# urbste/OpenImuCameraCalibrator

Measured on AMD Instinct MI355X. Metric: residual+Jacobian blocks/sec; wall-clock per LM iter, GoPro9 full calib, higher is better.
Workload: dtype f64

## Files before the change

openimucameracalibrator_amd/csrc/kernels_bcr.hip:

```cpp
#include <hip/hip_runtime.h>
#include <mutex>
#include <unordered_map>
#include "oicc_device.h"
#include "lm_decide.h"
#include "lm_launch.h"
#include "lm_retract.h"
#include "bcr_chain_body.h"
#include "../../include/oicc_hip.h"

namespace oicc {


struct BcrArgs {
  double* D;
  double* F;
  double* S;
  double* Lf;
  double* Mc;
  double* x;
  int32_t* fail;
  long long* prof;
  int n, a, Pb, rtf, LD;
  int delay;
  int o, s, p, m, pn;
// ... 8 lines not shown
#define BCR_RETURN_IF_DONE(A) do { if ((A).ctl != nullptr && (A).ctl->done != 0) return; } while (0)

__device__ __forceinline__ void bcr_lds_barrier() { asm volatile("s_waitcnt lgkmcnt(0)\n\ts_barrier" ::: "memory"); }
typedef double bcr_v4d __attribute__((ext_vector_type(4)));
typedef double bcr_v2d __attribute__((ext_vector_type(2)));

__device__ __forceinline__ void tri10(int t, int& xt, int& yt) {
  xt = t < 1 ? 0 : (t < 3 ? 1 : (t < 6 ? 2 : 3));
  yt = t - (xt * (xt + 1)) / 2;
}

struct BcrNoIdle { __device__ __forceinline__ void operator()() const {} };
template <int LD, class Idle = BcrNoIdle>
__device__ __forceinline__ void bcr_corner_solve(double* C, double* da, int* failp, int a, int tid, int wave, int lane, Idle idle = Idle()) {
  const int a1 = a + 1;
  if (a1 <= 16) {
    if (wave == 0) {
      double av[16], dinv = 0.0;
#pragma unroll
      for (int c = 0; c < 16; ++c) av[c] = (c < a && lane < a1 && lane >= c) ? C[c * LD + lane] : 0.0;
      bool bad = false;
#pragma unroll
      for (int c = 0; c < 16; ++c) {
        if (c < a) {
          const double piv = bcr_readlane(av[c], c);
          bad |= !(piv > 0.0);
          const double y0 = __builtin_amdgcn_rsq(piv);
          const double g0 = piv * y0, h0 = 0.5 * y0;
          const double r0 = fma(-g0, h0, 0.5);
          const double g1 = fma(g0, r0, g0), h1 = fma(h0, r0, h0);
          const double r1 = fma(-g1, h1, 0.5);
          const double u = (av[c] + av[c]) * h1;
          const double l = fma(u, r1, u);
          av[c] = l;
          if (lane == c) { const double y1 = h1 + h1; dinv = fma(y1, r1, y1); }
#pragma unroll
          for (int c2 = c + 1; c2 < 16; ++c2) {
            const double lc2 = bcr_readlane(l, c2);
            av[c2] = fma(-l, lc2, av[c2]);
          }
        }
      }
#pragma unroll
      for (int c = 0; c < 16; ++c) if (c < a && lane < a1 && lane >= c) C[c * LD + lane] = av[c];
      double lt[16];
#pragma unroll
      for (int q = 0; q < 16; ++q) lt[q] = (q < a && lane < q) ? C[lane * LD + q] : 0.0;
      double z = lane < a ? C[lane * LD + a] : 0.0, xq_mine = 0.0;
#pragma unroll
      for (int q = 15; q >= 0; --q) {
        if (q < a) {
          const double xq = bcr_readlane(z * dinv, q);
          if (lane == q) xq_mine = xq;
          z = fma(-lt[q], xq, z);
        }
      }
      if (lane < a) da[lane] = xq_mine;
      if (bad && lane == 0) *failp = 1;
    } else idle();
    __syncthreads();
    return;
  }
  if (wave == 0) {
    bool bad = false;
    for (int c = 0; c < a; ++c) {
      double* col = C + c * LD;
      const double mine = lane < a1 ? col[lane] : 0.0;
      double piv = bcr_readlane(mine, c);
      if (!(piv > 0.0)) { bad = true; piv = 1.0; }
      const double d = sqrt(piv);
      const double l = lane == c ? d : (lane > c ? mine / d : 0.0);
      if (lane >= c && lane < a1) col[lane] = l;
      for (int c2 = c + 1; c2 < a; ++c2) {
        const double l2 = bcr_readlane(l, c2);
        if (lane >= c2 && lane < a1) C[c2 * LD + lane] -= l * l2;
      }
    }
    if (bad && lane == 0) *failp = 1;
    double z = lane < a ? C[lane * LD + a] : 0.0;
    const double dc = lane < a ? 1.0 / C[lane * LD + lane] : 0.0;
    double xq_mine = 0.0;
    for (int q = a - 1; q >= 0; --q) {
      const double xq = bcr_readlane(z * dc, q);
      if (lane == q) xq_mine = xq;
      const double l = lane < q ? C[lane * LD + q] : 0.0;
      z = fma(-l, xq, z);
    }
    if (lane < a) da[lane] = xq_mine;
  } else idle();
  __syncthreads();
}

constexpr int kBackWaves = 8;
constexpr int kInvWaves = 16;
constexpr int kInvLD = 145;
constexpr int kInvMsDoubles = 3 * kChainStripDoubles;
constexpr int kInvDgRow = 128;

template <int XT>
__device__ __forceinline__ bcr_v4d bcri_z_tile(const double* W, int yt, int li, int lq) {
  constexpr int LD = kInvLD, K0 = 4 * XT, NK = 16 - K0;
  const double* py = W + lq * LD + 64 + 16 * yt + li;
  const double* px = W + lq * LD + 64 + 16 * XT + li;
  double vy[NK], vx[NK];
#pragma unroll
  for (int kk = 0; kk < NK; ++kk) { vy[kk] = py[4 * (K0 + kk) * LD]; vx[kk] = px[4 * (K0 + kk) * LD]; }
  asm volatile("" ::: "memory");
  bcr_v4d g = {0.0, 0.0, 0.0, 0.0}, g2 = {0.0, 0.0, 0.0, 0.0};
#pragma unroll
  for (int kk = 0; kk < NK; kk += 2) {
    g = __builtin_amdgcn_mfma_f64_16x16x4f64(vy[kk], vx[kk], g, 0, 0, 0);
    g2 = __builtin_amdgcn_mfma_f64_16x16x4f64(vy[kk + 1], vx[kk + 1], g2, 0, 0, 0);
  }
  g += g2;
  return g;
}

constexpr int kBackRows = 192 / kBackWaves;
struct BcrBackX {
  const double* xl; const double* xr; const double* xa;
  bool hasL, hasR;
  __device__ __forceinline__ double at(int r, int a) const {
    return r < 64 ? (hasL ? xl[r] : 0.0) : (r < 128 ? (hasR ? xr[r - 64] : 0.0) : (r < 128 + a ? xa[r - 128] : 0.0));
  }
};
__device__ __forceinline__ void bcri_back_rows(const double* Tg, int a, bool hasL, bool hasR, int w, int lane, double (&lv)[kBackRows], double& yv) {
#pragma unroll
  for (int k = 0; k < kBackRows; ++k) {
    const int r = w + kBackWaves * k;
    const bool ok = r < 128 + a && (hasL || r >= 64) && (hasR || r < 64 || r >= 128);
    lv[k] = ok ? Tg[r * 64 + lane] : 0.0;
  }
  yv = w == 0 ? Tg[(128 + a) * 64 + lane] : 0.0;
}
__device__ __forceinline__ double bcri_back_body(const double (&lv)[kBackRows], double yv, const BcrBackX& X, int a, double* part, bool active, int w, int lane) {
  if (active) {
    double sum = 0.0;
#pragma unroll
    for (int k = 0; k < kBackRows; ++k) { const int r = w + kBackWaves * k; sum = fma(lv[k], X.at(r, a), sum); }
    part[w * 64 + lane] = sum;
  }
  __syncthreads();
  double acc = 0.0;
  if (active && w == 0) {
#pragma unroll
    for (int ww = 0; ww < kBackWaves; ++ww) acc += part[ww * 64 + lane];
  }
  return yv - acc;
}

template <bool LAST, bool ZLDS, bool FOLD>
__device__ __forceinline__ void bcri_tail(const BcrArgs& A, double* W, double* da, int* failp, const double* Fs, const double* Cs, double* Zg, int tid, int wave, int lane, bool report, double* x0s) {
  static_assert(!FOLD || LAST, "the folded level follows the last block");
  constexpr int LD = kInvLD, NW = kInvWaves, NT = 64 * NW, FLD = 65;
  const int li = lane & 15, lq = lane >> 4;
  const int a = A.a, a1 = a + 1;
  const bool shared_writer = !FOLD || blockIdx.x == 0;
  double ttop[16], ytop = 0.0;
#pragma unroll
  for (int k = 0; k < 16; ++k) ttop[k] = 0.0;
  if (LAST && (A.top_l >= 0 || A.top_r >= 0)) {
    const int64_t ru64 = (int64_t)(192 + a1) * 64;
    const double* Tr = A.Lf + (A.top_r >= 0 ? A.top_r : 0) * ru64 + 4096;
    const double* Tl = A.Lf + (A.top_l >= 0 ? A.top_l : 0) * ru64 + 4096;
#pragma unroll
    for (int k = 0; k < 4; ++k) {
      const int r = wave + NW * k;
      if (A.top_r >= 0) { ttop[k] = Tr[r * 64 + lane]; if (r < A.a) ttop[4 + k] = Tr[(128 + r) * 64 + lane]; }
      if (A.top_l >= 0) { ttop[8 + k] = Tl[(64 + r) * 64 + lane]; if (r < A.a) ttop[12 + k] = Tl[(128 + r) * 64 + lane]; }
    }
    if (wave == 0 && A.top_r >= 0) ytop = Tr[(128 + A.a) * 64 + lane];
    if (wave == 1 && A.top_l >= 0) ytop = Tl[(128 + A.a) * 64 + lane];
    asm volatile("" ::: "memory");
  }
  for (int t = wave; t < 10; t += NW) {
    int xt, yt; tri10(t, xt, yt);
    const bcr_v4d g = xt == 0 ? bcri_z_tile<0>(W, yt, li, lq) : (xt == 1 ? bcri_z_tile<1>(W, yt, li, lq) : (xt == 2 ? bcri_z_tile<2>(W, yt, li, lq) : bcri_z_tile<3>(W, yt, li, lq)));
#pragma unroll
    for (int r = 0; r < 4; ++r) {
      const int x = 16 * xt + li, y = 16 * yt + lq + 4 * r;
      if (LAST || ZLDS) { W[y * LD + x] = g[r]; if (xt != yt) W[x * LD + y] = g[r]; }
      else { Zg[y * 64 + x] = g[r]; if (xt != yt) Zg[x * 64 + y] = g[r]; }
    }
  }
  __syncthreads();
  if (!LAST) {
    if (report && tid == 0 && *failp) atomicOr(A.fail, 1);
    return;
  }
  const int rtf = A.rtf;
  if (wave < 4 * rtf) {
    const int t = wave >> 2, w = wave & 3;
    const double* pf = Fs + lq * FLD + 16 * t + li;
    const double* pz = W + lq * LD + 16 * w + li;
    double vf[16], vz[16];
#pragma unroll
    for (int kk = 0; kk < 16; ++kk) { vf[kk] = pf[4 * kk * FLD]; vz[kk] = pz[4 * kk * LD]; }
    asm volatile("" ::: "memory");
    bcr_v4d tq = {0.0, 0.0, 0.0, 0.0};
#pragma unroll
    for (int kk = 0; kk < 16; ++kk) tq = __builtin_amdgcn_mfma_f64_16x16x4f64(vf[kk], vz[kk], tq, 0, 0, 0);
#pragma unroll
    for (int r = 0; r < 4; ++r) W[(16 * w + li) * LD + 64 + 16 * t + lq + 4 * r] = tq[r];
  }
  __syncthreads();
  if (wave < (rtf * (rtf + 1)) / 2) {
    int t1 = 0, u = wave; while (u >= t1 + 1) { u -= t1 + 1; ++t1; }
    const int t2 = u;
    const double* pt = W + lq * LD + 64 + 16 * t1 + li;
    const double* pf = Fs + lq * FLD + 16 * t2 + li;
    double vt[16], vf[16];
#pragma unroll
    for (int kk = 0; kk < 16; ++kk) { vt[kk] = pt[4 * kk * LD]; vf[kk] = pf[4 * kk * FLD]; }
    asm volatile("" ::: "memory");
    bcr_v4d g = {0.0, 0.0, 0.0, 0.0};
#pragma unroll
    for (int kk = 0; kk < 16; ++kk) g = __builtin_amdgcn_mfma_f64_16x16x4f64(vf[kk], vt[kk], g, 0, 0, 0);
#pragma unroll
    for (int r = 0; r < 4; ++r) { const int q1 = 16 * t1 + li, q2 = 16 * t2 + lq + 4 * r; if (q1 < a1 && q2 < a1) W[q2 * LD + q1] = Cs[q1 * a1 + q2] - g[r]; }
  }
  double lv[kBackRows], yv = 0.0;
#pragma unroll
  for (int k = 0; k < kBackRows; ++k) lv[k] = 0.0;
  constexpr int BW0 = NW - kBackWaves;
  int fi = 0; bool f_hasL = false, f_hasR = false;
  if (FOLD) {
    const int kp = 2 * (int)blockIdx.x + A.p;
    fi = A.o + kp * A.s; f_hasL = kp > 0; f_hasR = kp < A.m - 1;
  }
  __syncthreads();
  bcr_corner_solve<LD>(W, da, failp, a, tid, wave, lane, [&]() {
    if (FOLD && wave >= BW0) {
      bcri_back_rows(A.Lf + (int64_t)fi * (192 + a1) * 64 + 4096, a, f_hasL, f_hasR, wave - BW0, lane, lv, yv);
      asm volatile("" ::: "memory");
    }
  });
  if (shared_writer) for (int q = tid; q < a; q += NT) A.x[A.Pb + q] = da[q];
  if (wave == 0) {
    const double* tc = W + lane * LD + 64;
    double v = tc[a];
    for (int q = 0; q < a; q += 8) {
      double t8[8], d8[8];
#pragma unroll
      for (int k = 0; k < 8; ++k) { const bool ok = q + k < a; t8[k] = ok ? tc[q + k] : 0.0; d8[k] = ok ? da[q + k] : 0.0; }
#pragma unroll
      for (int k = 0; k < 8; ++k) v = fma(-t8[k], d8[k], v);
    }
    const int gi = A.last * 64 + lane;
    if (shared_writer && gi < A.Pb) A.x[gi] = v;
    x0s[lane] = gi < A.Pb ? v : 0.0;
  }
  __syncthreads();
  if (shared_writer && tid == 0 && *failp) atomicOr(A.fail, 1);
  if (A.top_l >= 0 || A.top_r >= 0) {
    double sum_r = 0.0, sum_l = 0.0;
#pragma unroll
    for (int k = 0; k < 4; ++k) {
      const int r = wave + NW * k;
      const double xn = x0s[r], xa = r < a ? da[r] : 0.0;
      sum_r = fma(ttop[k], xn, sum_r);     sum_r = fma(ttop[4 + k], xa, sum_r);
      sum_l = fma(ttop[8 + k], xn, sum_l); sum_l = fma(ttop[12 + k], xa, sum_l);
    }
    W[wave * 64 + lane] = sum_r;
    W[(NW + wave) * 64 + lane] = sum_l;
    __syncthreads();
    if (wave < 2) {
      const int blk = wave == 0 ? A.top_r : A.top_l;
      double acc = 0.0;
#pragma unroll
      for (int w = 0; w < NW; ++w) acc += W[(wave * NW + w) * 64 + lane];
      const int gi = blk * 64 + lane;
      const bool ok = blk >= 0 && gi < A.Pb;
      if (shared_writer && ok) A.x[gi] = ytop - acc;
      if (FOLD) x0s[64 * (1 + wave) + lane] = ok ? ytop - acc : 0.0;
    }
    if (FOLD) {
      __syncthreads();
      auto x_of = [&](int blk) -> const double* { return blk == A.last ? x0s : (blk == A.top_r ? x0s + 64 : x0s + 128); };
      BcrBackX X;
      X.hasL = f_hasL; X.hasR = f_hasR; X.xl = x_of(fi - A.s); X.xr = x_of(fi + A.s); X.xa = da;
      const double xv = bcri_back_body(lv, yv, X, a, W + 2 * NW * 64, wave >= BW0, wave - BW0, lane);
      const int gi = fi * 64 + lane;
      if (wave == BW0 && gi < A.Pb) A.x[gi] = xv;
    }
  }
}


struct BcrNoPark { __device__ __forceinline__ void operator()(double*) const {} };
template <bool LAST, bool PROF, bool ZLDS = false, bool FOLD = false, class LoadD, class Park = BcrNoPark>
__device__ __forceinline__ void bcri_invert_body(const BcrArgs& A, const int i, LoadD load_d, const bool report = true, Park park = Park()) {
  constexpr int LD = kInvLD, NW = kInvWaves, NT = 64 * NW, NTILE = 20, SLOTS = (NTILE + NW - 1) / NW, RU = 128, NAW = 3, FLD = 65;
  static_assert(NW == 16, "the corner phases of block 0 take one tile per wave");
  extern __shared__ __attribute__((aligned(16))) double lds[];
  const int tid = threadIdx.x, lane = tid & 63;
  const int wave = __builtin_amdgcn_readfirstlane(tid >> 6);
  const int li = lane & 15, lq = lane >> 4;
  double* const W = lds;
  double* const da = W + 64 * LD;
  int* const failp = reinterpret_cast<int*>(da + 64);
  double* const ms = da + 64 + 8;
  static_assert(kInvMsDoubles >= NAW * kChainStripDoubles && (kChainStripDoubles * 8) % 16 == 0 && kInvMsDoubles >= 256 && ((64 * LD + 64 + 8) * 8) % 16 == 0, "ms");
  double* const Fs = ms + kInvMsDoubles;
  double* const Cs = Fs + 64 * FLD;
  const int a1 = A.a + 1;
  double* Zg = A.Lf + (int64_t)i * (192 + a1) * 64;
  const double* Fg = A.F + (int64_t)i * 64 * a1;
  const double* Sf = (LAST && A.side != 0) ? Zg + 4096 : nullptr;
  const double* Sm = (LAST && A.side != 0) ? Zg + 4096 + 64 * a1 : nullptr;
  const bool prof = PROF && A.prof != nullptr && blockIdx.x == 0 && wave == 0;
  long long pc[8] = {0, 0, 0, 0, 0, 0, 0, 0};
  long long tprev = prof ? clock64() : 0;
#define BCR_MARK(k) do { if (PROF && prof) { const long long tn_ = clock64(); pc[k] += tn_ - tprev; tprev = tn_; } } while (0)
  if (tid == 0) *failp = 0;
  {
    constexpr int PER = 4096 / NT;
    double gd[PER], gf[PER], gc[PER];
#pragma unroll
    for (int k = 0; k < PER; ++k) {
      const int e = tid + k * NT;
      gd[k] = load_d(e);
      if (LAST) { const int c = e >> 6, q = e & 63; gf[k] = q < a1 ? Fg[c * a1 + q] + (Sf != nullptr ? Sf[c * a1 + q] : 0.0) : 0.0; }
      if (LAST) gc[k] = e < a1 * a1 ? A.Mc[e] + (Sm != nullptr ? Sm[e] : 0.0) : 0.0;
    }
#pragma unroll
    for (int k = 0; k < PER; ++k) {
      const int e = tid + k * NT;
      const int c = e >> 6, r = e & 63;
      W[c * LD + r] = r >= c ? gd[k] : 0.0;
      if (c < 16 && r < 16) W[c * LD + kInvDgRow + r] = r >= c ? gd[k] : 0.0;
      W[c * LD + 64 + r] = r == c ? 1.0 : 0.0;
      if (LAST) Fs[c * FLD + r] = gf[k];
      if (LAST && e < a1 * a1) Cs[e] = gc[k];
    }
    park(Fs);
  }
  __syncthreads();
  int t_rt[SLOTS], t_ct[SLOTS]; bool t_ok[SLOTS];
  bcr_v4d acc[SLOTS];
#pragma unroll
  for (int k = 0; k < SLOTS; ++k) {
    const int t = wave + NW * k;
    t_ok[k] = t < NTILE;
    int xt, yt; tri10(t < 10 ? t : (t < NTILE ? t - 10 : 0), xt, yt);
    if (t < 10) { t_rt[k] = xt; t_ct[k] = yt; } else { t_rt[k] = 4 + yt; t_ct[k] = xt; }
    const double* src = W + (16 * t_ct[k] + lq) * LD + 16 * t_rt[k] + li;
    acc[k][0] = src[0]; acc[k][1] = src[4 * LD]; acc[k][2] = src[8 * LD]; acc[k][3] = src[12 * LD];
  }
  BCR_MARK(0);
  const int prow = 16 + wave * 48 + (lane - 16);
  for (int p = 0; p < 4; ++p) {
    const int j0 = 16 * p;
    if (wave < NAW) {
      const int rho = lane < 16 ? j0 + lane : prow;
      const bool act = lane < 16 || (rho >= j0 + 16 && rho < RU && !(rho >= 64 && rho - 64 > j0 + 15));
      if (A.delay > 0 && wave > 0) for (int k = 0; k < A.delay; ++k) __builtin_amdgcn_s_sleep(16);
      const double* colp = W + j0 * LD + (lane < 16 ? kInvDgRow + lane : (act ? rho : 0));
      double av[16];
#pragma unroll
      for (int c = 0; c < 16; ++c) av[c] = colp[c * LD];
      if (PROF && prof) { asm volatile("s_waitcnt lgkmcnt(0)" ::: "memory"); }
      BCR_MARK(6);
      const bool bad = bcr_chain_panel<kChainSchedule>(av, ms + wave * kChainStripDoubles + lane, ms + wave * kChainStripDoubles);
      if (PROF && prof) { asm volatile("s_nop 0" :: "v"(av[15])); }
      BCR_MARK(7);
      if (act && (lane >= 16 || wave == 0)) {
        double* cp = W + j0 * LD + rho;
#pragma unroll
        for (int c = 0; c < 16; ++c) cp[c * LD] = av[c];
      }
      if (bad && lane == 0) *failp = 1;
    }
    BCR_MARK(1);
    bcr_lds_barrier();
    BCR_MARK(2);
    if (p < 3) {
#pragma unroll
      for (int k = 0; k < SLOTS; ++k) {
        if (t_ok[k] && t_ct[k] > p && (t_rt[k] < 4 || t_rt[k] - 4 <= p)) {
          const double* pa = W + (j0 + lq) * LD + 16 * t_ct[k] + li;
          const double* pb = W + (j0 + lq) * LD + 16 * t_rt[k] + li;
          double va[4], vb[4];
#pragma unroll
          for (int kq = 0; kq < 4; ++kq) { va[kq] = pa[4 * kq * LD]; vb[kq] = -pb[4 * kq * LD]; }
#pragma unroll
          for (int kq = 0; kq < 4; ++kq) acc[k] = __builtin_amdgcn_mfma_f64_16x16x4f64(va[kq], vb[kq], acc[k], 0, 0, 0);
          if (t_ct[k] == p + 1) {
            double* dst = W + (16 * t_ct[k] + lq) * LD + 16 * t_rt[k] + li;
            dst[0] = acc[k][0]; dst[4 * LD] = acc[k][1]; dst[8 * LD] = acc[k][2]; dst[12 * LD] = acc[k][3];
            if (t_rt[k] == t_ct[k]) {
              double* dd = W + (16 * t_ct[k] + lq) * LD + kInvDgRow + li;
              dd[0] = li >= lq ? acc[k][0] : 0.0; dd[4 * LD] = li >= lq + 4 ? acc[k][1] : 0.0; dd[8 * LD] = li >= lq + 8 ? acc[k][2] : 0.0; dd[12 * LD] = li >= lq + 12 ? acc[k][3] : 0.0;
            }
          }
        }
      }
    }
    BCR_MARK(3);
    bcr_lds_barrier();
    BCR_MARK(4);
  }
  BCR_MARK(4);
  bcri_tail<LAST, ZLDS, FOLD>(A, W, da, failp, Fs, Cs, Zg, tid, wave, lane, report, ms);
  BCR_MARK(5);
  if (PROF && prof && lane == 0) for (int k = 0; k < 8; ++k) A.prof[k] = pc[k];
#undef BCR_MARK
}

template <bool LAST, bool PROF>
__global__ __launch_bounds__(64 * kInvWaves) void bcri_invert_kernel(BcrArgs A) {
  BCR_RETURN_IF_DONE(A);
  const int i = LAST ? A.last : A.o + A.s * (2 * (int)blockIdx.x + A.p);
  const double* Dg = A.D + (int64_t)i * 4096;
  const double* Sd = (LAST && A.side != 0) ? A.Lf + (int64_t)i * (192 + A.a + 1) * 64 : nullptr;
  bcri_invert_body<LAST, PROF>(A, i, [Dg, Sd](int e) { double v = Dg[e]; if (LAST && Sd != nullptr && (e & 63) >= (e >> 6)) v += Sd[e]; return v; });
}

__global__ __launch_bounds__(64 * kInvWaves) void bcri_last_backward_kernel(BcrArgs A) {
  BCR_RETURN_IF_DONE(A);
  const int i = A.last;
  const double* Dg = A.D + (int64_t)i * 4096;
  const double* Sd = A.side != 0 ? A.Lf + (int64_t)i * (192 + A.a + 1) * 64 : nullptr;
  bcri_invert_body<true, false, false, true>(A, i, [Dg, Sd](int e) { double v = Dg[e]; if (Sd != nullptr && (e & 63) >= (e >> 6)) v += Sd[e]; return v; });
}

struct BcrSchurGroup {
  int k, i, irs;
  bool hasL, hasR, ghostR;
  int xk, xt, yk, ny;
  bool store_t;
  bool leaves;
};
__device__ __forceinline__ BcrSchurGroup bcri_schur_group(const BcrArgs& A, int g, int piv) {
  BcrSchurGroup G;
  const int rtf = A.rtf;
  G.k = 2 * piv + A.p;
  G.i = A.o + G.k * A.s;
  G.hasL = G.k > 0;
  G.ghostR = A.ghost != 0 && G.k == A.m - 1;
  G.hasR = G.k < A.m - 1 || G.ghostR;
  G.irs = G.ghostR ? A.n : G.i + A.s;
  if (g < 4) { G.xk = 0; G.xt = g; G.yk = 0; G.ny = g + 1; G.store_t = true; }
  else if (g < 8) { G.xk = 1; G.xt = g - 4; G.yk = 0; G.ny = 4; G.store_t = false; }
  else if (g < 12) { G.xk = 1; G.xt = g - 8; G.yk = 1; G.ny = G.xt + 1; G.store_t = true; }
  else { g -= 12; G.yk = g / rtf; G.xt = g - G.yk * rtf; G.xk = 2; G.ny = G.yk < 2 ? 4 : G.xt + 1; G.store_t = G.yk == (G.hasL ? 0 : 1); }
  G.leaves = ((G.xk == 1 || G.yk == 1) && !G.hasR) || ((G.xk == 0 || G.yk == 0) && !G.hasL);
  return G;
}
struct BcrSchurGlobalOps {
  static constexpr bool kLateY = false;
  const double *px, *pz, *py; int sx, sy; bool okx, oky;
  __device__ __forceinline__ double x(int kk) const { return px[4 * kk * sx]; }
  __device__ __forceinline__ double z(int kk) const { return pz[4 * kk * 64]; }
  __device__ __forceinline__ double y(int kk) const { return oky ? py[4 * kk * sy] : 0.0; }
};
struct BcrSchurLdsOps {
  static constexpr bool kLateY = true;
  const double *px, *pz, *py; bool okx;
  __device__ __forceinline__ double x(int kk) const { return px[64 * kk]; }
  __device__ __forceinline__ double z(int kk) const { return pz[4 * kk * kInvLD]; }
  __device__ __forceinline__ double y(int kk) const { return py[64 * kk]; }
};
template <class Ops>
__device__ __forceinline__ void bcri_schur_body(const BcrArgs& A, const BcrSchurGroup& G, double (*Ts)[68], const Ops& ops, const bool active, const int wave, const int lane) {
  const int li = lane & 15, lq = lane >> 4;
  const int a1 = A.a + 1, s = A.s;
  const int k = G.k, i = G.i, il = i - s, irs = G.irs, xk = G.xk, xt = G.xt, yk = G.yk, ny = G.ny;
  const bool hasL = G.hasL, ghostR = G.ghostR, store_t = G.store_t, okx = ops.okx;
  double* Tg = A.Lf + (int64_t)i * (192 + a1) * 64 + 4096;
  double vx[16], vz[16], vy[16];
  if (active) {
#pragma unroll
    for (int kk = 0; kk < 16; ++kk) { vx[kk] = ops.x(kk); vz[kk] = ops.z(kk); }
    if (!Ops::kLateY) {
#pragma unroll
      for (int kk = 0; kk < 16; ++kk) vy[kk] = ops.y(kk);
    }
    asm volatile("" ::: "memory");
    bcr_v4d tq = {0.0, 0.0, 0.0, 0.0}, tq2 = {0.0, 0.0, 0.0, 0.0};
#pragma unroll
    for (int kk = 0; kk < 16; kk += 2) {
      tq = __builtin_amdgcn_mfma_f64_16x16x4f64(okx ? vx[kk] : 0.0, vz[kk], tq, 0, 0, 0);
      tq2 = __builtin_amdgcn_mfma_f64_16x16x4f64(okx ? vx[kk + 1] : 0.0, vz[kk + 1], tq2, 0, 0, 0);
    }
    tq += tq2;
    const int trow0 = xk == 0 ? 16 * xt : (xk == 1 ? 64 + 16 * xt : 128 + 16 * xt);
#pragma unroll
    for (int r = 0; r < 4; ++r) {
      const int row = lq + 4 * r;
      Ts[row][16 * wave + li] = tq[r];
      if (store_t && (xk != 2 || 16 * xt + row < a1)) Tg[(int64_t)(trow0 + row) * 64 + 16 * wave + li] = tq[r];
    }
  }
  __syncthreads();
  if (!active || wave >= ny) return;
  const int yt = wave;
  const int kn = hasL ? (k - 2 + A.p) / 2 : 0;
  const bool il_is_pivot = (kn & 1) == A.pn;
  const bool swap = xk == 1 && yk == 0 && !il_is_pivot && !ghostR;
  double vt[16];
  if (Ops::kLateY) {
#pragma unroll
    for (int kk = 0; kk < 16; ++kk) vy[kk] = ops.y(kk);
  }
#pragma unroll
  for (int kk = 0; kk < 16; ++kk) vt[kk] = Ts[li][4 * kk + lq];
  asm volatile("" ::: "memory");
  bcr_v4d gq = {0.0, 0.0, 0.0, 0.0}, gq2 = {0.0, 0.0, 0.0, 0.0};
  if (swap) {
#pragma unroll
    for (int kk = 0; kk < 16; kk += 2) {
      gq = __builtin_amdgcn_mfma_f64_16x16x4f64(vt[kk], vy[kk], gq, 0, 0, 0);
      gq2 = __builtin_amdgcn_mfma_f64_16x16x4f64(vt[kk + 1], vy[kk + 1], gq2, 0, 0, 0);
    }
  } else {
#pragma unroll
    for (int kk = 0; kk < 16; kk += 2) {
      gq = __builtin_amdgcn_mfma_f64_16x16x4f64(vy[kk], vt[kk], gq, 0, 0, 0);
      gq2 = __builtin_amdgcn_mfma_f64_16x16x4f64(vy[kk + 1], vt[kk + 1], gq2, 0, 0, 0);
    }
  }
  gq += gq2;
  const int ils = hasL ? il : i;
  double* Dl = A.D + (int64_t)ils * 4096; double* Dr = A.D + (int64_t)irs * 4096;
  double* Fl = A.F + (int64_t)ils * 64 * a1; double* Fr = A.F + (int64_t)irs * 64 * a1;
  double* So = A.S + (A.offS_out + kn) * 4096;
  const bool to_side = A.side != 0 && !hasL;
  double* Sd = A.Lf + (int64_t)irs * (192 + a1) * 64;
#pragma unroll
  for (int r = 0; r < 4; ++r) {
    const double v = -gq[r];
    if (xk == 1 && yk == 0) {
      if (!swap) { const int x = 16 * xt + li, y = 16 * yt + lq + 4 * r; So[y * 64 + x] = v; }
      else       { const int y = 16 * yt + li, x = 16 * xt + lq + 4 * r; So[x * 64 + y] = v; }
    } else if (xk < 2) {
      const int x = 16 * xt + li, y = 16 * yt + lq + 4 * r;
      if (to_side) { if (x >= y) Sd[y * 64 + x] = v; }
      else if (x >= y && v != 0.0) unsafeAtomicAdd((xk == 0 ? Dl : Dr) + y * 64 + x, v);
    } else if (yk < 2) {
      const int q = 16 * xt + li, y = 16 * yt + lq + 4 * r;
      if (to_side) { if (q < a1) Sd[4096 + y * a1 + q] = v; }
      else if (q < a1 && v != 0.0) unsafeAtomicAdd((yk == 0 ? Fl : Fr) + y * a1 + q, v);
    } else {
      const int q1 = 16 * xt + li, q2 = 16 * yt + lq + 4 * r;
      if (to_side) { if (q1 < a1 && q2 <= q1) { Sd[4096 + 64 * a1 + q1 * a1 + q2] = v; Sd[4096 + 64 * a1 + q2 * a1 + q1] = v; } }
      else if (q1 < a1 && q2 <= q1 && v != 0.0) {
        unsafeAtomicAdd(A.Mc + q1 * a1 + q2, v);
        if (q1 != q2) unsafeAtomicAdd(A.Mc + q2 * a1 + q1, v);
      }
    }
  }
}

__global__ __launch_bounds__(256) void bcri_schur_kernel(BcrArgs A) {
  BCR_RETURN_IF_DONE(A);
  __shared__ double Ts[16][68];
  const int tid = threadIdx.x, lane = tid & 63;
  const int wave = __builtin_amdgcn_readfirstlane(tid >> 6);
  const int li = lane & 15, lq = lane >> 4;
  const int a1 = A.a + 1;
  if ((int)blockIdx.y == (int)gridDim.y - 1 && A.carry > 0) {
    const int m = A.carry;
    const double* src = A.S + (A.offS_in + (m - 1)) * 4096; double* dst = A.S + (A.offS_out + (m - 1) / 2) * 4096;
    for (int e = (int)blockIdx.x * 256 + tid; e < 4096; e += (int)gridDim.x * 256) dst[e] = src[e];
    return;
  }
  const BcrSchurGroup G = bcri_schur_group(A, (int)blockIdx.x, (int)blockIdx.y);
  if (G.leaves) return;
  const double* SL = A.S + (A.offS_in + (G.hasL ? G.k - 1 : 0)) * 4096;
  const double* SR = A.S + (A.offS_in + G.k) * 4096;
  const double* Fg = A.F + (int64_t)G.i * 64 * a1;
  const double* Zg = A.Lf + (int64_t)G.i * (192 + a1) * 64;
  auto border_ptr = [&](int kind, int t, int& stride, bool& ok) -> const double* {
    if (kind == 0) { stride = 64; ok = true; return SL + lq * 64 + 16 * t + li; }
    if (kind == 1) { stride = 64; ok = true; return SR + lq * 64 + 16 * t + li; }
    const int q = 16 * t + li; ok = q < a1; stride = a1; return Fg + lq * a1 + (ok ? q : 0);
  };
  BcrSchurGlobalOps ops;
  ops.px = border_ptr(G.xk, G.xt, ops.sx, ops.okx);
  ops.py = border_ptr(G.yk, wave < G.ny ? wave : 0, ops.sy, ops.oky);
  ops.pz = Zg + lq * 64 + 16 * wave + li;
  bcri_schur_body(A, G, Ts, ops, true, wave, lane);
}

constexpr int kInvLdsDoubles = 64 * kInvLD + 64 + 8 + kInvMsDoubles;
constexpr int kJoinLdsDoubles = kInvLdsDoubles + 5 * 1024 + 16 * 68;
__global__ __launch_bounds__(64 * kInvWaves) void bcri_invert_schur_kernel(BcrArgs A) {
  BCR_RETURN_IF_DONE(A);
  const BcrSchurGroup G = bcri_schur_group(A, (int)blockIdx.x, (int)blockIdx.y);
  if (G.leaves) return;
  const int tid = threadIdx.x, lane = tid & 63;
  const int wave = __builtin_amdgcn_readfirstlane(tid >> 6);
  const int li = lane & 15, lq = lane >> 4;
  const int a1 = A.a + 1;
  const double* SL = A.S + (A.offS_in + (G.hasL ? G.k - 1 : 0)) * 4096;
  const double* SR = A.S + (A.offS_in + G.k) * 4096;
  const double* Fg = A.F + (int64_t)G.i * 64 * a1;
  const int kv = tid >> 4, l = tid & 15;
  auto border_at = [&](int kind, int t) -> double {
    if (kind == 0) return SL[kv * 64 + 16 * t + l];
    if (kind == 1) return SR[kv * 64 + 16 * t + l];
    const int q = 16 * t + l; return q < a1 ? Fg[kv * a1 + q] : 0.0;
  };
  double bx = border_at(G.xk, G.xt), by[4];
#pragma unroll
  for (int t = 0; t < 4; ++t) by[t] = t < G.ny ? border_at(G.yk, t) : 0.0;
  asm volatile("" ::: "memory");
  const double* Dg = A.D + (int64_t)G.i * 4096;
  const bool report = (int)blockIdx.x == (G.hasL ? 0 : 8);
  bcri_invert_body<false, false, true>(A, G.i, [Dg](int e) { return Dg[e]; }, report,
    [&](double* P) {
      P[tid] = bx;
#pragma unroll
      for (int t = 0; t < 4; ++t) P[1024 * (1 + t) + tid] = by[t];
    });
  extern __shared__ __attribute__((aligned(16))) double lds[];
  const double* W = lds;
  const double* P = lds + kInvLdsDoubles;
  double (*Ts)[68] = reinterpret_cast<double (*)[68]>(lds + kInvLdsDoubles + 5 * 1024);
  const bool active = wave < 4;
  BcrSchurLdsOps ops;
  ops.okx = true;
  ops.px = P + lq * 16 + li;
  ops.py = P + 1024 * (1 + (active && wave < G.ny ? wave : 0)) + lq * 16 + li;
  ops.pz = W + lq * kInvLD + 16 * (active ? wave : 0) + li;
  bcri_schur_body(A, G, Ts, ops, active, wave, lane);
}

struct BcrOwn {
  int e = -1, code = -1;
  double sc0 = 0.0, d2 = 0.0, g = 0.0;
  const double* x = nullptr; double* xc = nullptr;
};
constexpr int kRetractPark = 12;
template <int NB>
__device__ __forceinline__ BcrOwn bcr_retract_claim(const BcrArgs& A, const RetractReq& R, const SolveBuffers& sb, int b_lo, int b_hi, bool arrow_wg, int tid) {
  BcrOwn o; o.x = R.x; o.xc = R.xc;
  NormalEq ne = R.ne;
  if (A.ctl != nullptr) { o.x = A.ctl->xp[0]; o.xc = A.ctl->xp[1]; ne.base = A.ctl->nep[0]; }
  const int e_hi = b_hi * 64 < A.Pb ? b_hi * 64 : A.Pb;
  if (tid < 64 * NB) { const int e = b_lo * 64 + tid; if (e < e_hi) o.e = e; }
  else if (tid < 64 * NB + A.a && arrow_wg) o.e = A.Pb + (tid - 64 * NB);
  if (o.e >= 0) { o.code = R.rmap[o.e]; o.sc0 = sb.scale[o.e]; o.d2 = sb.D2[o.e]; o.g = ne.g()[o.e]; }
  return o;
}
__device__ __forceinline__ int bcr_rm_steps(int kind) { return kind == kRmEucl ? 1 : (kind == kRmTic ? 6 : 3); }
__device__ __forceinline__ int bcr_rm_params(int kind) { return kind == kRmEucl ? 1 : (kind == kRmTic ? 7 : (kind == kRmSo3 || kind == kRmPt ? 4 : 3)); }
__device__ __forceinline__ void bcr_retract_park(const SolveBuffers& sb, const BcrOwn& o, double* rpark, int stride, int tid) {
  if (o.code < 0) return;
  const int kind = o.code & 7; const int64_t po = o.code >> 3;
  const int nd = bcr_rm_steps(kind), np = bcr_rm_params(kind);
  for (int c = 0; c < np; ++c) rpark[c * stride + tid] = o.x[po + c];
  for (int c = 1; c < nd; ++c) rpark[(6 + c) * stride + tid] = sb.scale[o.e + c];
}
template <int OW>
__device__ __forceinline__ void bcr_retract_finish(const BcrArgs& A, const RetractReq& R, const SolveBuffers& sb, const BcrOwn& o, const double* xflat, int e_base,
                                                   const double* xarrow, const double* rpark, int stride, double* red, int tid, int wave, int lane) {
  __syncthreads();
  if (blockIdx.x == 0 && tid == 0) {
    if (A.ctl != nullptr) { if (A.ctl->stamps != nullptr && A.ctl->seq < A.ctl->trace_cap) A.ctl->stamps[3 * A.ctl->seq + 1] = wall_clock64(); }
    else *R.ne.cost() = 0.0;
  }
  double step_sq = 0.0, x_sq = 0.0, model = 0.0;
  if (o.e >= 0) {
    auto step_at = [&](int e) { return e >= A.Pb ? xarrow[e - A.Pb] : xflat[e - e_base]; };
    model = lm_model_term(step_at(o.e), o.d2, o.g, o.sc0);
    if (o.code >= 0) {
      const int kind = o.code & 7;
      const double alpha = R.alpha;
      const int nd = bcr_rm_steps(kind), np = bcr_rm_params(kind);
      double d[6], sc[6], pv[7];
#pragma unroll
      for (int c = 0; c < 6; ++c) { d[c] = c < nd ? step_at(o.e + c) : 0.0; sc[c] = c == 0 ? o.sc0 : (c < nd ? rpark[(6 + c) * stride + tid] : 0.0); }
#pragma unroll
      for (int c = 0; c < 7; ++c) pv[c] = c < np ? rpark[c * stride + tid] : 0.0;
      double* out = o.xc + (o.code >> 3);
      if (kind == kRmSo3) lm_store_so3(lm_retract_so3(Quat{pv[0], pv[1], pv[2], pv[3]}, d, sc, alpha), pv, out, step_sq, x_sq);
      else if (kind == kRmEucl) lm_retract_eucl(pv[0], d[0], sc[0], alpha, out, step_sq, x_sq);
      else if (kind == kRmAb || kind == kRmGb) { const double bound = kind == kRmAb ? R.max_ab : R.max_gb; for (int c = 0; c < 3; ++c) lm_retract_box(pv[c], d[c], sc[c], alpha, bound, out + c, step_sq, x_sq); }
      else if (kind == kRmPt) lm_retract_point(pv, d, sc, alpha, out, step_sq, x_sq);
      else if (kind == kRmTic) lm_retract_tic(pv, d, sc, alpha, out, step_sq, x_sq);
    }
  }
  if (wave < OW) {
#pragma unroll
    for (int off = 32; off > 0; off >>= 1) { step_sq += __shfl_xor(step_sq, off); x_sq += __shfl_xor(x_sq, off); model += __shfl_xor(model, off); }
    if (lane == 0) { red[wave] = step_sq; red[64 + wave] = x_sq; red[128 + wave] = model; }
  }
  __syncthreads();
  if (tid < 3) {
    double acc = 0.0;
    for (int w = 0; w < OW; ++w) acc += red[64 * tid + w];
    unsafeAtomicAdd(tid == 0 ? &sb.st->step_norm_sq : (tid == 1 ? &sb.st->x_norm_sq : &sb.st->model_cost_change), acc);
  }
}

__global__ __launch_bounds__(64 * kBackWaves) void bcri_backward_kernel(BcrArgs A) {
  BCR_RETURN_IF_DONE(A);
  __shared__ double xs[192];
  __shared__ double part[kBackWaves][64];
  const int tid = threadIdx.x, lane = tid & 63;
  const int wave = __builtin_amdgcn_readfirstlane(tid >> 6);
  const int a = A.a, a1 = a + 1, s = A.s;
  const int kp = 2 * (int)blockIdx.x + A.p;
  const int i = A.o + kp * s, il = i - s;
  const bool hasL = kp > 0;
  const bool hasR = kp < A.m - 1 || A.ghost != 0;
  const int ir = kp < A.m - 1 ? i + s : A.n;
  double lv[kBackRows], yv;
  bcri_back_rows(A.Lf + (int64_t)i * (192 + a1) * 64 + 4096, a, hasL, hasR, wave, lane, lv, yv);
  double xin = 0.0;
  if (tid < 64) { const int gi = il * 64 + tid; xin = (hasL && gi < A.Pb) ? A.x[gi] : 0.0; }
  else if (tid < 128) { const int gi = ir * 64 + (tid - 64); xin = (hasR && gi < A.Pb) ? A.x[gi] : 0.0; }
  else if (tid < 128 + a) xin = A.x[A.Pb + (tid - 128)];
  if (tid < 192) xs[tid] = xin;
  __syncthreads();
  BcrBackX X;
  X.xl = xs; X.xr = xs + 64; X.xa = xs + 128; X.hasL = true; X.hasR = true;
  const double xv = bcri_back_body(lv, yv, X, a, &part[0][0], true, wave, lane);
  const int gi = i * 64 + lane;
  if (wave == 0 && gi < A.Pb) A.x[gi] = xv;
}

template <bool RETRACT>
__device__ __forceinline__ void bcri_backward2_body(const BcrArgs& A, int ou, int pu, int mu, int npiv_upper, int orphan_l, int orphan_r, const RetractReq& R, const SolveBuffers& sb) {
  constexpr int NW = 16, RW1 = 192 / NW, RW2 = 192 / (NW / 2);
  __shared__ double xw[6][64];
  __shared__ double part[NW][64];
  double* const xs0 = xw[0]; double* const xs1 = xw[2]; double* const xs2 = xw[4]; double* const xs3 = xw[5];
  const int tid = threadIdx.x, lane = tid & 63;
  const int wave = __builtin_amdgcn_readfirstlane(tid >> 6);
  const int a = A.a, a1 = a + 1, s = A.s, n = A.n;
  const int64_t ru64 = (int64_t)(192 + a1) * 64;
  const int lone_ix = (int)blockIdx.x - npiv_upper;
  const bool lone = lone_ix >= 0;
  const bool lone_l = lone && orphan_l >= 0 && lone_ix == 0, lone_r = lone && !lone_l;
  const int ku = 2 * (int)blockIdx.x + pu;
  const int j = lone_l ? orphan_l - s : (lone_r ? orphan_r + s : ou + ku * 2 * s);
  const int jl = j - 2 * s, jr = j + 2 * s;
  const bool ghost = A.ghost != 0;
  const bool has_jl = lone_r || (!lone && ku > 0);
  const bool has_jr = lone_l || (!lone && (ku < mu - 1 || ghost));
  const int jrs = (!lone && ku == mu - 1) ? n : jr;
  const int half = wave >> 3, hw = wave & 7;
  const int ci = half == 0 ? j - s : j + s;
  const bool child = lone ? (half == 0 ? lone_r : lone_l) : (half == 0 ? ci >= A.o : ci <= A.o + (A.m - 1) * s);
  const bool child_hasL = half == 0 ? has_jl : !lone;
  const bool child_hasR = half == 0 ? (!lone || ghost) : has_jr;
  auto xin = [&](int blk, int r) { const int gi = blk * 64 + r; return gi < A.Pb ? A.x[gi] : 0.0; };
  if (tid < 64) xs0[tid] = has_jl ? xin(jl, tid) : 0.0;
  else if (tid < 128) xs2[tid - 64] = has_jr ? xin(jrs, tid - 64) : 0.0;
  else if (tid < 192) xs3[tid - 128] = tid - 128 < a ? A.x[A.Pb + (tid - 128)] : 0.0;
  else if (tid < 256 && lone) xs1[tid - 192] = (lone_r && ghost) ? xin(n, tid - 192) : 0.0;
  __shared__ double rpark[RETRACT ? kRetractPark : 1][384];
  BcrOwn own;
  if (RETRACT) {
    const int b_lo = j - 2 > 0 ? j - 2 : 0;
    int b_hi = j + 2 < n ? j + 2 : n;
    if (!lone && (int)blockIdx.x == npiv_upper - 1 && orphan_r < 0) b_hi = n;
    own = bcr_retract_claim<5>(A, R, sb, b_lo, b_hi, blockIdx.x == 0, tid);
  }
  double l1[RW1], l2[RW2], y1 = 0.0, y2 = 0.0;
  {
    const double* T1 = A.Lf + (lone ? 0 : j) * ru64 + 4096;
#pragma unroll
    for (int k = 0; k < RW1; ++k) {
      const int r = wave + NW * k;
      const bool ok = !lone && r < 128 + a && (has_jl || r >= 64) && (has_jr || r < 64 || r >= 128);
      l1[k] = ok ? T1[r * 64 + lane] : 0.0;
    }
    if (wave == 0 && !lone) y1 = T1[(128 + a) * 64 + lane];
    const double* T2 = A.Lf + (child ? ci : 0) * ru64 + 4096;
#pragma unroll
    for (int k = 0; k < RW2; ++k) {
      const int r = hw + 8 * k;
      const bool ok = child && r < 128 + a && (child_hasL || r >= 64) && (child_hasR || r < 64 || r >= 128);
      l2[k] = ok ? T2[r * 64 + lane] : 0.0;
    }
    if (hw == 0 && child) y2 = T2[(128 + a) * 64 + lane];
// ... 512 lines not shown
```

Before: 57.85 million.

## Compute Schur T product from inverse factors, overlapping partial tiles with chain phases

In the fused invert+Schur kernel, the explicit symmetric Z write to LDS is skipped. The T = X·Z product is instead formed from the triangular inverse factors in LDS as 10 chunk tiles. Idle waves compute some chunks during the panel phases of the inversion (a shadow callback), and a staged pass finishes the rest. This aims to hide the T-stage MFMA work under the serial chain panels and to drop the Z-tile writes and a barrier stage. It adds LDS scratch for partial tiles plus summation on read, and it reorders floating-point accumulation.

```diff
diff --git a/openimucameracalibrator_amd/csrc/kernels_bcr.hip b/openimucameracalibrator_amd/csrc/kernels_bcr.hip
--- a/openimucameracalibrator_amd/csrc/kernels_bcr.hip
+++ b/openimucameracalibrator_amd/csrc/kernels_bcr.hip
@@ -184,6 +184,11 @@
 template <bool LAST, bool ZLDS, bool FOLD>
 __device__ __forceinline__ void bcri_tail(const BcrArgs& A, double* W, double* da, int* failp, const double* Fs, const double* Cs, double* Zg, int tid, int wave, int lane, bool report, double* x0s) {
   static_assert(!FOLD || LAST, "the folded level follows the last block");
+  static_assert(!ZLDS || !LAST, "the last block keeps Z");
+  if (ZLDS) {
+    if (report && tid == 0 && *failp) atomicOr(A.fail, 1);
+    return;
+  }
   constexpr int LD = kInvLD, NW = kInvWaves, NT = 64 * NW, FLD = 65;
   const int li = lane & 15, lq = lane >> 4;
   const int a = A.a, a1 = a + 1;
@@ -211,7 +216,7 @@
 #pragma unroll
     for (int r = 0; r < 4; ++r) {
       const int x = 16 * xt + li, y = 16 * yt + lq + 4 * r;
-      if (LAST || ZLDS) { W[y * LD + x] = g[r]; if (xt != yt) W[x * LD + y] = g[r]; }
+      if (LAST) { W[y * LD + x] = g[r]; if (xt != yt) W[x * LD + y] = g[r]; }
       else { Zg[y * 64 + x] = g[r]; if (xt != yt) Zg[x * 64 + y] = g[r]; }
     }
   }
@@ -320,8 +325,9 @@
 
 
 struct BcrNoPark { __device__ __forceinline__ void operator()(double*) const {} };
-template <bool LAST, bool PROF, bool ZLDS = false, bool FOLD = false, class LoadD, class Park = BcrNoPark>
-__device__ __forceinline__ void bcri_invert_body(const BcrArgs& A, const int i, LoadD load_d, const bool report = true, Park park = Park()) {
+struct BcrNoShadow { __device__ __forceinline__ void operator()(int) const {} };
+template <bool LAST, bool PROF, bool ZLDS = false, bool FOLD = false, class LoadD, class Park = BcrNoPark, class Shadow = BcrNoShadow>
+__device__ __forceinline__ void bcri_invert_body(const BcrArgs& A, const int i, LoadD load_d, const bool report = true, Park park = Park(), Shadow shadow = Shadow()) {
   constexpr int LD = kInvLD, NW = kInvWaves, NT = 64 * NW, NTILE = 20, SLOTS = (NTILE + NW - 1) / NW, RU = 128, NAW = 3, FLD = 65;
   static_assert(NW == 16, "the corner phases of block 0 take one tile per wave");
   extern __shared__ __attribute__((aligned(16))) double lds[];
@@ -402,6 +408,8 @@
         for (int c = 0; c < 16; ++c) cp[c * LD] = av[c];
       }
       if (bad && lane == 0) *failp = 1;
+    } else if (ZLDS && p > 0) {
+      shadow(p - 1);
     }
     BCR_MARK(1);
     bcr_lds_barrier();
@@ -480,51 +488,58 @@
   return G;
 }
 struct BcrSchurGlobalOps {
+  static constexpr bool kTStage = true;
   static constexpr bool kLateY = false;
   const double *px, *pz, *py; int sx, sy; bool okx, oky;
   __device__ __forceinline__ double x(int kk) const { return px[4 * kk * sx]; }
   __device__ __forceinline__ double z(int kk) const { return pz[4 * kk * 64]; }
   __device__ __forceinline__ double y(int kk) const { return oky ? py[4 * kk * sy] : 0.0; }
+  __device__ __forceinline__ double t(const double (*Ts)[68], int kk, int li, int lq) const { return Ts[li][4 * kk + lq]; }
 };
 struct BcrSchurLdsOps {
+  static constexpr bool kTStage = false;
   static constexpr bool kLateY = true;
-  const double *px, *pz, *py; bool okx;
-  __device__ __forceinline__ double x(int kk) const { return px[64 * kk]; }
-  __device__ __forceinline__ double z(int kk) const { return pz[4 * kk * kInvLD]; }
+  const double *py, *TP;
   __device__ __forceinline__ double y(int kk) const { return py[64 * kk]; }
+  __device__ __forceinline__ double t(const double (*)[68], int kk, int li, int lq) const;
 };
+__device__ __forceinline__ int bcri_schur_trow0(const BcrSchurGroup& G) { return G.xk == 0 ? 16 * G.xt : (G.xk == 1 ? 64 + 16 * G.xt : 128 + 16 * G.xt); }
 template <class Ops>
 __device__ __forceinline__ void bcri_schur_body(const BcrArgs& A, const BcrSchurGroup& G, double (*Ts)[68], const Ops& ops, const bool active, const int wave, const int lane) {
   const int li = lane & 15, lq = lane >> 4;
   const int a1 = A.a + 1, s = A.s;
   const int k = G.k, i = G.i, il = i - s, irs = G.irs, xk = G.xk, xt = G.xt, yk = G.yk, ny = G.ny;
-  const bool hasL = G.hasL, ghostR = G.ghostR, store_t = G.store_t, okx = ops.okx;
-  double* Tg = A.Lf + (int64_t)i * (192 + a1) * 64 + 4096;
-  double vx[16], vz[16], vy[16];
-  if (active) {
-#pragma unroll
-    for (int kk = 0; kk < 16; ++kk) { vx[kk] = ops.x(kk); vz[kk] = ops.z(kk); }
-    if (!Ops::kLateY) {
-#pragma unroll
-      for (int kk = 0; kk < 16; ++kk) vy[kk] = ops.y(kk);
-    }
-    asm volatile("" ::: "memory");
-    bcr_v4d tq = {0.0, 0.0, 0.0, 0.0}, tq2 = {0.0, 0.0, 0.0, 0.0};
-#pragma unroll
-    for (int kk = 0; kk < 16; kk += 2) {
-      tq = __builtin_amdgcn_mfma_f64_16x16x4f64(okx ? vx[kk] : 0.0, vz[kk], tq, 0, 0, 0);
-      tq2 = __builtin_amdgcn_mfma_f64_16x16x4f64(okx ? vx[kk + 1] : 0.0, vz[kk + 1], tq2, 0, 0, 0);
-    }
-    tq += tq2;
-    const int trow0 = xk == 0 ? 16 * xt : (xk == 1 ? 64 + 16 * xt : 128 + 16 * xt);
-#pragma unroll
-    for (int r = 0; r < 4; ++r) {
-      const int row = lq + 4 * r;
-      Ts[row][16 * wave + li] = tq[r];
-      if (store_t && (xk != 2 || 16 * xt + row < a1)) Tg[(int64_t)(trow0 + row) * 64 + 16 * wave + li] = tq[r];
-    }
-  }
-  __syncthreads();
+  const bool hasL = G.hasL, ghostR = G.ghostR;
+  double vy[16];
+  if constexpr (Ops::kTStage) {
+    const bool store_t = G.store_t, okx = ops.okx;
+    double* Tg = A.Lf + (int64_t)i * (192 + a1) * 64 + 4096;
+    double vx[16], vz[16];
+    if (active) {
+#pragma unroll
+      for (int kk = 0; kk < 16; ++kk) { vx[kk] = ops.x(kk); vz[kk] = ops.z(kk); }
+      if (!Ops::kLateY) {
+#pragma unroll
+        for (int kk = 0; kk < 16; ++kk) vy[kk] = ops.y(kk);
+      }
+      asm volatile("" ::: "memory");
+      bcr_v4d tq = {0.0, 0.0, 0.0, 0.0}, tq2 = {0.0, 0.0, 0.0, 0.0};
+#pragma unroll
+      for (int kk = 0; kk < 16; kk += 2) {
+        tq = __builtin_amdgcn_mfma_f64_16x16x4f64(okx ? vx[kk] : 0.0, vz[kk], tq, 0, 0, 0);
+        tq2 = __builtin_amdgcn_mfma_f64_16x16x4f64(okx ? vx[kk + 1] : 0.0, vz[kk + 1], tq2, 0, 0, 0);
+      }
+      tq += tq2;
+      const int trow0 = bcri_schur_trow0(G);
+#pragma unroll
+      for (int r = 0; r < 4; ++r) {
+        const int row = lq + 4 * r;
+        Ts[row][16 * wave + li] = tq[r];
+        if (store_t && (xk != 2 || 16 * xt + row < a1)) Tg[(int64_t)(trow0 + row) * 64 + 16 * wave + li] = tq[r];
+      }
+    }
+    __syncthreads();
+  }
   if (!active || wave >= ny) return;
   const int yt = wave;
   const int kn = hasL ? (k - 2 + A.p) / 2 : 0;
@@ -536,7 +551,7 @@
     for (int kk = 0; kk < 16; ++kk) vy[kk] = ops.y(kk);
   }
 #pragma unroll
-  for (int kk = 0; kk < 16; ++kk) vt[kk] = Ts[li][4 * kk + lq];
+  for (int kk = 0; kk < 16; ++kk) vt[kk] = ops.t(Ts, kk, li, lq);
   asm volatile("" ::: "memory");
   bcr_v4d gq = {0.0, 0.0, 0.0, 0.0}, gq2 = {0.0, 0.0, 0.0, 0.0};
   if (swap) {
@@ -615,8 +630,144 @@
   bcri_schur_body(A, G, Ts, ops, true, wave, lane);
 }
 
+constexpr int kTxChunks = 10, kTxStride = 17, kTxTileDoubles = 16 * kTxStride;
+__device__ __forceinline__ int bcri_tx_chunk(int p, int q) { return (p * (p + 1)) / 2 + q; }
+__device__ __forceinline__ double* bcri_tx_ytile(double* W, int t) { return W + 16 * (t & 3) * kInvLD + 16 * (t >> 2); }
+template <int T0>
+__device__ __forceinline__ void bcri_tx_stage(double* W, const double* P, double* TP, const int wave, const int lane) {
+  constexpr int LD = kInvLD;
+  const int li = lane & 15, lq = lane >> 4;
+  const int chunk = wave + T0;
+  int p, q; tri10(chunk < kTxChunks ? chunk : 0, p, q);
+  if (chunk < kTxChunks) {
+    const double* pb = P + (16 * q + lq) * 16 + li;
+    const double* px = W + (16 * p + li) * LD + 64 + 16 * q + lq;
+    double vb[4], vx[4];
+#pragma unroll
+    for (int kk = 0; kk < 4; ++kk) { vb[kk] = pb[64 * kk]; vx[kk] = px[4 * kk]; }
+    asm volatile("" ::: "memory");
+    bcr_v4d y = {0.0, 0.0, 0.0, 0.0};
+#pragma unroll
+    for (int kk = 0; kk < 4; ++kk) y = __builtin_amdgcn_mfma_f64_16x16x4f64(vb[kk], vx[kk], y, 0, 0, 0);
+    double* yp = bcri_tx_ytile(W, chunk) + li * LD + lq;
+#pragma unroll
+    for (int r = 0; r < 4; ++r) yp[4 * r] = y[r];
+  }
+  bcr_lds_barrier();
+  if (chunk < kTxChunks) {
+    const int i = q, c0 = bcri_tx_chunk(p, 0);
+    const double* px = W + (16 * p + lq) * LD + 64 + 16 * i + li;
+    double yv[4][4], vx[4];
+#pragma unroll
+    for (int qq = 0; qq < 4; ++qq) {
+      if (qq <= p) {
+        const double* yp = bcri_tx_ytile(W, c0 + qq) + lq * LD + li;
+#pragma unroll
+        for (int kk = 0; kk < 4; ++kk) yv[qq][kk] = yp[4 * kk * LD];
+      } else {
+#pragma unroll
+        for (int kk = 0; kk < 4; ++kk) yv[qq][kk] = 0.0;
+      }
+    }
+#pragma unroll
+    for (int kk = 0; kk < 4; ++kk) vx[kk] = px[4 * kk * LD];
+    asm volatile("" ::: "memory");
+    bcr_v4d t = {0.0, 0.0, 0.0, 0.0};
+#pragma unroll
+    for (int kk = 0; kk < 4; ++kk) {
+      double ys = yv[0][kk];
+#pragma unroll
+      for (int qq = 1; qq < 4; ++qq) if (qq <= p) ys += yv[qq][kk];
+      t = __builtin_amdgcn_mfma_f64_16x16x4f64(ys, vx[kk], t, 0, 0, 0);
+    }
+    double* tp = TP + chunk * kTxTileDoubles + li * kTxStride + lq;
+#pragma unroll
+    for (int r = 0; r < 4; ++r) tp[4 * r] = t[r];
+  }
+  bcr_lds_barrier();
+}
+__device__ __forceinline__ void bcri_tx_shadow(const double* W, const double* P, double* TP, double* YS, const int pp, const int wave, const int lane) {
+  constexpr int LD = kInvLD;
+  if (wave != 3 + 4 * pp) return;
+  const int li = lane & 15, lq = lane >> 4;
+  double* ys = YS + pp * kTxTileDoubles;
+  {
+    const double* pb = P + lq * 16 + li;
+    const double* px = W + (16 * pp + li) * LD + 64 + lq;
+    double vb[3][4], vx[3][4];
+#pragma unroll
+    for (int q = 0; q < 3; ++q) {
+#pragma unroll
+      for (int kk = 0; kk < 4; ++kk) { vb[q][kk] = q <= pp ? pb[256 * q + 64 * kk] : 0.0; vx[q][kk] = q <= pp ? px[16 * q + 4 * kk] : 0.0; }
+    }
+    asm volatile("" ::: "memory");
+    bcr_v4d y = {0.0, 0.0, 0.0, 0.0};
+#pragma unroll
+    for (int q = 0; q < 3; ++q) {
+      if (q <= pp) {
+        bcr_v4d yq = {0.0, 0.0, 0.0, 0.0};
+#pragma unroll
+        for (int kk = 0; kk < 4; ++kk) yq = __builtin_amdgcn_mfma_f64_16x16x4f64(vb[q][kk], vx[q][kk], yq, 0, 0, 0);
+        if (q == 0) y = yq; else y += yq;
+      }
+    }
+#pragma unroll
+    for (int r = 0; r < 4; ++r) ys[li * kTxStride + lq + 4 * r] = y[r];
+  }
+  bcr_wave_sync();
+  {
+    const double* px = W + (16 * pp + lq) * LD + 64 + li;
+    double vy[4], vx[3][4];
+#pragma unroll
+    for (int kk = 0; kk < 4; ++kk) vy[kk] = ys[(4 * kk + lq) * kTxStride + li];
+#pragma unroll
+    for (int i = 0; i < 3; ++i) {
+#pragma unroll
+      for (int kk = 0; kk < 4; ++kk) vx[i][kk] = i <= pp ? px[4 * kk * LD + 16 * i] : 0.0;
+    }
+    asm volatile("" ::: "memory");
+#pragma unroll
+    for (int i = 0; i < 3; ++i) {
+      if (i <= pp) {
+        bcr_v4d t = {0.0, 0.0, 0.0, 0.0};
+#pragma unroll
+        for (int kk = 0; kk < 4; ++kk) t = __builtin_amdgcn_mfma_f64_16x16x4f64(vy[kk], vx[i][kk], t, 0, 0, 0);
+        double* tp = TP + bcri_tx_chunk(pp, i) * kTxTileDoubles + li * kTxStride + lq;
+#pragma unroll
+        for (int r = 0; r < 4; ++r) tp[4 * r] = t[r];
+      }
+    }
+  }
+}
+template <int I>
+__device__ __forceinline__ double bcri_tx_sum(const double* TP, int row, int cl) {
+  const double* tp = TP + cl * kTxStride + row;
+  double v = tp[bcri_tx_chunk(I, I) * kTxTileDoubles];
+#pragma unroll
+  for (int p = I + 1; p < 4; ++p) v += tp[bcri_tx_chunk(p, I) * kTxTileDoubles];
+  return v;
+}
+__device__ __forceinline__ double bcri_tx_at(const double* TP, int i, int row, int cl) {
+  return i == 0 ? bcri_tx_sum<0>(TP, row, cl) : (i == 1 ? bcri_tx_sum<1>(TP, row, cl) : (i == 2 ? bcri_tx_sum<2>(TP, row, cl) : bcri_tx_sum<3>(TP, row, cl)));
+}
+__device__ __forceinline__ double BcrSchurLdsOps::t(const double (*)[68], int kk, int li, int lq) const { return bcri_tx_at(TP, kk >> 2, li, 4 * (kk & 3) + lq); }
+__device__ __forceinline__ void bcri_tx_store(const BcrArgs& A, const BcrSchurGroup& G, const double* TP, const int w, const int lane) {
+  const int li = lane & 15, lq = lane >> 4;
+  const int a1 = A.a + 1;
+  double* Tg = A.Lf + (int64_t)G.i * (192 + a1) * 64 + 4096;
+  const int trow0 = bcri_schur_trow0(G);
+  double v[4];
+#pragma unroll
+  for (int r = 0; r < 4; ++r) v[r] = bcri_tx_at(TP, w, lq + 4 * r, li);
+#pragma unroll
+  for (int r = 0; r < 4; ++r) {
+    const int row = lq + 4 * r;
+    if (G.xk != 2 || 16 * G.xt + row < a1) Tg[(int64_t)(trow0 + row) * 64 + 16 * w + li] = v[r];
+  }
+}
+
 constexpr int kInvLdsDoubles = 64 * kInvLD + 64 + 8 + kInvMsDoubles;
-constexpr int kJoinLdsDoubles = kInvLdsDoubles + 5 * 1024 + 16 * 68;
+constexpr int kJoinLdsDoubles = kInvLdsDoubles + 5 * 1024 + (kTxChunks + 3) * kTxTileDoubles;
 __global__ __launch_bounds__(64 * kInvWaves) void bcri_invert_schur_kernel(BcrArgs A) {
   BCR_RETURN_IF_DONE(A);
   const BcrSchurGroup G = bcri_schur_group(A, (int)blockIdx.x, (int)blockIdx.y);
@@ -639,24 +790,26 @@
   for (int t = 0; t < 4; ++t) by[t] = t < G.ny ? border_at(G.yk, t) : 0.0;
   asm volatile("" ::: "memory");
   const double* Dg = A.D + (int64_t)G.i * 4096;
+  extern __shared__ __attribute__((aligned(16))) double lds_[];
   const bool report = (int)blockIdx.x == (G.hasL ? 0 : 8);
   bcri_invert_body<false, false, true>(A, G.i, [Dg](int e) { return Dg[e]; }, report,
     [&](double* P) {
       P[tid] = bx;
 #pragma unroll
       for (int t = 0; t < 4; ++t) P[1024 * (1 + t) + tid] = by[t];
-    });
+    },
+    [&](int pp) { bcri_tx_shadow(lds_, lds_ + kInvLdsDoubles, lds_ + kInvLdsDoubles + 5 * 1024, lds_ + kInvLdsDoubles + 5 * 1024 + kTxChunks * kTxTileDoubles, pp, wave, lane); });
   extern __shared__ __attribute__((aligned(16))) double lds[];
-  const double* W = lds;
+  double* W = lds;
   const double* P = lds + kInvLdsDoubles;
-  double (*Ts)[68] = reinterpret_cast<double (*)[68]>(lds + kInvLdsDoubles + 5 * 1024);
+  double* TP = lds + kInvLdsDoubles + 5 * 1024;
+  bcri_tx_stage<6>(W, P, TP, wave, lane);
+  if (G.store_t && wave >= 4 && wave < 8) bcri_tx_store(A, G, TP, wave - 4, lane);
   const bool active = wave < 4;
   BcrSchurLdsOps ops;
-  ops.okx = true;
-  ops.px = P + lq * 16 + li;
+  ops.TP = TP;
   ops.py = P + 1024 * (1 + (active && wave < G.ny ? wave : 0)) + lq * 16 + li;
-  ops.pz = W + lq * kInvLD + 16 * (active ? wave : 0) + li;
-  bcri_schur_body(A, G, Ts, ops, active, wave, lane);
+  bcri_schur_body(A, G, nullptr, ops, active, wave, lane);
 }
 
 struct BcrOwn {
```

Result: faster. 58.80 million, median of 6 (+1.6%).
